# SUTD-MDQS/QILaplace.jl

Measured on AMD Instinct MI355X. Metric: MPO×MPS site-contractions/sec + max |coeff err|, n=24 χ_s=64 χ_c=128, higher is better.
Workload: dtype f64; 1 GPU; zt_n24_chi64_D128; sites=48, mps_bonds_max=64, mpo_bonds_max=128, parallelism=replicas x1 (one signal per GPU), ranks_reported_by_collective_backend=1

## Files before the change

### qilaplace.jl_amd/csrc/qil_internal.h

```cpp
#pragma once

#include <hip/hip_runtime.h>
#include <hip/hip_complex.h>

#include <cstdint>
#include <cstdio>
#include <cstring>
#include <functional>
#include <map>
#include <condition_variable>
#include <mutex>
#include <set>
#include <string>
#include <vector>

#include "qilaplace_hip.h"
#include "qilaplace_hip_testing.h"

#include <atomic>

struct qil_lds_grant {
    static constexpr int kDevices = 64;
    std::atomic<size_t> bytes[kDevices] = {};
    hipError_t ensure(int device, const void* fn, size_t want) {
// ... 125 lines not shown
void qil_comm_orphan(struct qil_comm* cm);
void qil_ctx_transfer(qil_context* from, qil_context* to, void* p);
void qil_chain_rebind(struct qil_chain* c, qil_context* to);
int qil_mps_clone_to(qil_context* ctx, const struct qil_mps* psi, struct qil_mps** out);

static inline size_t qil_elem_size(int dtype) { return dtype == QIL_C64 ? 16 : 8; }

struct qil_chain {
    qil_context* ctx = nullptr;
    int dtype = QIL_F64;
    int paired = 0;
    int phys_rank = 1;
    std::vector<int64_t> dims;
    std::vector<int64_t> site_ids;
    std::vector<void*> site;
    double amplitude = 1.0;
    qil_chain() = default;
    qil_chain(const qil_chain&) = delete;
    qil_chain& operator=(const qil_chain&) = delete;
    ~qil_chain() {
        if (ctx) ctx->chains.erase(this);
    }
    int64_t n() const { return (int64_t)site.size(); }
    int64_t site_elems(int64_t i) const {
        return dims[i] * (phys_rank == 1 ? 2 : 4) * dims[i + 1];
    }
    size_t site_bytes(int64_t i) const { return (size_t)site_elems(i) * qil_elem_size(dtype); }
};
struct qil_mps : qil_chain {};
struct qil_mpo : qil_chain {};

int qil_chain_alloc(qil_context* ctx, qil_chain* c, int64_t n, int dtype, int paired, int phys_rank,
                    const int64_t* bond_dims, const int64_t* site_ids);
int qil_chain_release(qil_chain* c);
void qil_chain_bind(qil_chain* c, qil_context* ctx);
int qil_chain_set_site(qil_chain* c, int64_t i, void* p, int64_t dl, int64_t dr);
void qil_chain_adopt(qil_chain* c, int64_t i, void* p);

unsigned qil_fail_count();
struct qil_call_scope {
    qil_context* ctx;
    uint64_t serial0;
    unsigned fails0;
    explicit qil_call_scope(qil_context* c);
    ~qil_call_scope();
    qil_call_scope(const qil_call_scope&) = delete;
    qil_call_scope& operator=(const qil_call_scope&) = delete;
};

int qil_dev_right_envs(const struct qil_mps* psi, const char* verb, void** Rall, std::vector<long long>& roff, double* log_norm2);

int qil_dev_gemm(qil_context* ctx, int dtype, int opA, int opB, int64_t m, int64_t n, int64_t k,
                 const void* A, int64_t lda, const void* B, int64_t ldb, void* C, int64_t ldc);
int qil_dev_gemm_skinny(qil_context* ctx, int dtype, int opA, int opB, int64_t m, int64_t n, int64_t k,
                        const void* A, int64_t lda, const void* B, int64_t ldb, void* C, int64_t ldc);
struct qil_gemm_batch {
    int64_t count = 1;
    int64_t a_bs = 0, b_bs = 0, c_bs = 0;
    const uint8_t* b_sel = nullptr;
    int64_t b_sel_step = 0, b_sel_stride = 0;
};
int qil_dev_gemm_batched(qil_context* ctx, int dtype, int opA, int opB, int64_t m, int64_t n, int64_t k,
                         const void* A, int64_t lda, const void* B, int64_t ldb, void* C, int64_t ldc,
                         const qil_gemm_batch* batch);
struct qil_gemm_problem {
    const void* A;
    const void* B;
    void* C;
    int m, n, k;
    int lda, ldb, ldc;
    int tile_begin;
    int pad;
};
int qil_dev_gemm_grouped(qil_context* ctx, int dtype, std::vector<qil_gemm_problem>& probs);
bool qil_dev_gemm_grouped_fits(size_t nproblems);
int qil_check_pair(const char* verb, const struct qil_mps* phi, const struct qil_mps* psi);
int qil_sum_compress_impl(qil_context* ctx, const struct qil_mps* const* terms, int64_t nb, const double* w, int odt,
                          int64_t maxdim, double tol, int sweeps, int64_t zip_maxdim, struct qil_mps** out);
int qil_dev_diag_abs2(qil_context* ctx, int dtype, const void* R, int64_t ldr, int64_t n, double* host_out);
int qil_dev_transpose(qil_context* ctx, int dtype, int conj, int64_t m, int64_t n, const void* A, int64_t lda,
                      void* At, int64_t ldt);
int qil_dev_svd(qil_context* ctx, int dtype, int64_t m, int64_t n, void* A, int64_t lda, void* U,
                int64_t ldu, double* S_host, void* Vh, int64_t ldvh, double negligible_rel = 0.0);
int qil_dev_svd_left(qil_context* ctx, int dtype, int64_t p, int64_t q, void* B, int64_t ldb, void* Uiso, int64_t ldu,
                     double* S_host, void* SVh, int64_t ldsvh, double negligible_rel, int* handled, double cert_cutoff = 0.0,
                     double deflate = 0.0);
int qil_dev_qr_certified(qil_context* ctx, int dtype, int64_t m, int64_t n, const void* A, int64_t lda, double cutoff, void* Qout,
                         void* Rout, bool* certified);
int qil_dev_set_identity(qil_context* ctx, int dtype, void* V, int64_t ldv, int64_t n);
int qil_dev_qr_positive(qil_context* ctx, int dtype, int64_t m, int64_t n, void* A, int64_t lda,
                        void* R, int64_t ldr, bool orthonormal = false);
int qil_dev_copy2d(qil_context* ctx, void* dst, size_t dpitch, const void* src, size_t spitch, size_t width, size_t height);
int qil_dev_copy(qil_context* ctx, void* dst, const void* src, size_t bytes);
int qil_dev_zero2d(qil_context* ctx, void* dst, size_t pitch, size_t width, size_t height);
int qil_dev_zero(qil_context* ctx, void* dst, size_t bytes);
int64_t qil_truncation_rank(const double* S, int64_t n, double cutoff, bool use_cutoff, int64_t maxdim,
                            int64_t mindim);
int qil_dev_scale(qil_context* ctx, int dtype, int side, int64_t m, int64_t n, void* A, int64_t lda,
                  const double* s_host);
int qil_dev_fill_normal(qil_context* ctx, int dtype, void* p, int64_t n_elems, uint64_t seed,
                        double scale);
```

### qilaplace.jl_amd/csrc/qil_linalg.hip

```cpp
#include <algorithm>
#include <chrono>
#include <cmath>
#include <cstring>
#include <numeric>
#include <utility>

#include "qil_internal.h"
#include "qil_launch.h"
#include "qil_device_utils.h"

namespace {

using namespace qil_dev;

constexpr int GK = 16;
#ifndef QIL_GEMM_GAUSS
#define QIL_GEMM_GAUSS 1
#endif
#ifndef QIL_GEMM_PAD
#define QIL_GEMM_PAD 2
#endif
constexpr int GPAD = QIL_GEMM_PAD;
typedef double d4 __attribute__((ext_vector_type(4)));

__device__ __forceinline__ void put_plane(double* S0, double* S1, int off, double v) {
    S0[off] = v;
    (void)S1;
}
__device__ __forceinline__ void put_plane(double* S0, double* S1, int off, c64 v) {
    S0[off] = v.re;
    S1[off] = v.im;
}
__device__ __forceinline__ double maybe_conj(double v, int) { return v; }
__device__ __forceinline__ c64 maybe_conj(c64 v, int cj) { return cj ? c64{v.re, -v.im} : v; }

template <class T, int BM, int BN, int WM, int WN, bool PIPE, bool ARC, bool BKC, int GKT = GK, int DEEP = 0>
__device__ __forceinline__ void gemm_mfma_body(const uint3 blockIdx, const uint3 gridDim, long long m, long long n, long long k_total,
                                                 const T* __restrict__ A, long long a_rs, long long a_ks, int conjA,
                                                 const T* __restrict__ B, long long b_ks, long long b_cs, int conjB,
                                                 T* __restrict__ C, long long ldc, long long kchunk,
                                                 long long cstride, int tiles_m, int tiles_n, int col_fastest,
                                                 long long a_bs, long long b_bs, long long c_bs,
                                                 const int* __restrict__ cmap, int cmap_blk,
                                                 const uint8_t* __restrict__ b_sel, long long b_sel_step,
                                                 long long b_sel_stride, int subtract) {
    constexpr bool CX = sizeof(T) == 16;
    constexpr int NP = CX ? 2 : 1;
    constexpr int LA = BM + GPAD, LB = BN + GPAD;
    constexpr int NBUF = PIPE ? 2 : 1;
    constexpr int TM = WM / 16, TN = WN / 16;
    constexpr int EA = BM * GKT / 256, EB = BN * GKT / 256;
    static_assert((BM / WM) * (BN / WN) == 4, "4 waves per workgroup");
    extern __shared__ __attribute__((aligned(16))) char gemm_smem[];
    double* As = reinterpret_cast<double*>(gemm_smem);
    double* Bs = As + NBUF * NP * GKT * LA;
    const int tid = threadIdx.x;
    const int lane = tid & 63, wave = tid >> 6;
    const int wr = (wave % (BM / WM)) * WM, wc = (wave / (BM / WM)) * WN;
    const int l15 = lane & 15, l4 = lane >> 4;
    int tile = blockIdx.x;
    if (col_fastest & 2) tile = (tile % 8) * (tiles_m * tiles_n / 8) + tile / 8;
    int tm, tn;
    if (col_fastest & 1) {
        tn = tile % tiles_n;
        tm = tile / tiles_n;
    } else {
        tm = tile % tiles_m;
        tn = tile / tiles_m;
    }
    const long long row0 = (long long)tm * BM, col0 = (long long)tn * BN;
    const long long kbeg = (long long)blockIdx.z * kchunk;
    const long long kend = min(k_total, kbeg + kchunk);
    A += (long long)blockIdx.y * a_bs;
    B += (long long)blockIdx.y * b_bs;
    if (b_sel) B += (long long)b_sel[(long long)blockIdx.y * b_sel_step] * b_sel_stride;
    C += (long long)blockIdx.z * cstride + (long long)blockIdx.y * c_bs;
    if (cmap) cmap += (long long)blockIdx.y * (n / cmap_blk);

    d4 rr[TM][TN], ii[CX ? TM : 1][CX ? TN : 1], ri[CX ? TM : 1][CX ? TN : 1];
#pragma unroll
    for (int a = 0; a < TM; ++a)
#pragma unroll
        for (int b = 0; b < TN; ++b) {
            rr[a][b] = d4{0, 0, 0, 0};
            if (CX) {
                ii[a][b] = d4{0, 0, 0, 0};
                ri[a][b] = d4{0, 0, 0, 0};
            }
        }
    constexpr bool a_rows_contig = ARC, b_k_contig = BKC;
    T ra[EA], rb[EB];
    const T* pa[EA];
    const T* pb[EB];
    int ka[EA], kb[EB], sa[EA], sb[EB];
#pragma unroll
    for (int e = 0; e < EA; ++e) {
        const int idx = tid + 256 * e;
        const int i = a_rows_contig ? idx % BM : idx / GKT;
// ... 90 lines not shown
                for (int ti = 0; ti < TM; ++ti)
#pragma unroll
                    for (int tj = 0; tj < TN; ++tj) {
                        rr[ti][tj] = __builtin_amdgcn_mfma_f64_16x16x4f64(bre[tj], are[ti], rr[ti][tj], 0, 0, 0);
                        if constexpr (CX) {
                            ii[ti][tj] = __builtin_amdgcn_mfma_f64_16x16x4f64(bim[tj], aim[ti], ii[ti][tj], 0, 0, 0);
                            ri[ti][tj] = __builtin_amdgcn_mfma_f64_16x16x4f64(bim[tj], are[ti], ri[ti][tj], 0, 0, 0);
                            ri[ti][tj] = __builtin_amdgcn_mfma_f64_16x16x4f64(bre[tj], aim[ti], ri[ti][tj], 0, 0, 0);
                        }
                    }
            }
        }
    };
    if constexpr (PIPE && DEEP) {
        T ra1[EA], rb1[EB];
        if (kbeg < kend) load_tile_into(ra, rb, kbeg);
        if (kbeg + GKT < kend) load_tile_into(ra1, rb1, kbeg + GKT);
        for (long long k0 = kbeg; k0 < kend; k0 += 2 * GKT) {
            store_tile_from(ra, rb, 0, k0);
            __syncthreads();
            if (k0 + 2 * GKT < kend) load_tile_into(ra, rb, k0 + 2 * GKT);
            mfma_tile(0);
            if (k0 + GKT >= kend) break;
            store_tile_from(ra1, rb1, 1, k0 + GKT);
            __syncthreads();
            if (k0 + 3 * GKT < kend) load_tile_into(ra1, rb1, k0 + 3 * GKT);
            mfma_tile(1);
        }
    } else {
        int buf = 0;
        if (PIPE && kbeg < kend) load_tile(kbeg);
        for (long long k0 = kbeg; k0 < kend; k0 += GKT) {
            if (!PIPE) {
                if (k0 > kbeg) __syncthreads();
                load_tile(k0);
            }
            store_tile(buf, k0);
            __syncthreads();
            if (PIPE && k0 + GKT < kend) load_tile(k0 + GKT);
            mfma_tile(buf);
            if (PIPE) buf ^= 1;
        }
    }
#pragma unroll
    for (int ti = 0; ti < TM; ++ti)
#pragma unroll
        for (int tj = 0; tj < TN; ++tj)
#pragma unroll
            for (int r = 0; r < 4; ++r) {
                const long long gr = row0 + wr + 16 * ti + l15;
                const long long gc = col0 + wc + 16 * tj + l4 + 4 * r;
                if (gr < m && gc < n) {
                    const long long oc = cmap ? (long long)cmap[gc / cmap_blk] * cmap_blk + gc % cmap_blk : gc;
                    double* cp = reinterpret_cast<double*>(C + gr + ldc * oc);
                    if (subtract) {
                        if (CX) {
                            cp[0] -= rr[ti][tj][r] - ii[ti][tj][r];
                            cp[1] -= QIL_GEMM_GAUSS ? rr[ti][tj][r] + ri[ti][tj][r] : ri[ti][tj][r];
                        } else {
                            cp[0] -= rr[ti][tj][r];
                        }
                    } else if (CX) {
                        cp[0] = rr[ti][tj][r] - ii[ti][tj][r];
                        cp[1] = QIL_GEMM_GAUSS ? rr[ti][tj][r] + ri[ti][tj][r] : ri[ti][tj][r];
                    } else {
                        cp[0] = rr[ti][tj][r];
                    }
                }
            }
}
template <class T, int BM, int BN, int WM, int WN, bool PIPE, bool ARC, bool BKC, int GKT = GK, int DEEP = 0>
struct gemm_mfma_k {
    static constexpr int NT = 256, MINW = (DEEP ? 1 : (BM * BN <= 128 * 128 ? 2 : 1));
    template <class... QA>
    static __device__ __forceinline__ void run(const uint3 b, const uint3 g, QA... a) {
        gemm_mfma_body<T, BM, BN, WM, WN, PIPE, ARC, BKC, GKT, DEEP>(b, g, a...);
    }
};

template <class T>
__device__ __forceinline__ void splitk_reduce_body(const uint3 blockIdx, const uint3 gridDim, const T* __restrict__ W, long long cstride, int splits, long long m, long long n,
                              T* __restrict__ C, long long ldc, int subtract) {
    for (long long t = blockIdx.x * (long long)blockDim.x + threadIdx.x; t < m * n;
         t += (long long)gridDim.x * blockDim.x) {
        T acc = W[t];
        for (int z = 1; z < splits; ++z) acc = add_t(acc, W[t + z * cstride]);
        T* cp = C + (t % m) + ldc * (t / m);
        *cp = subtract ? sub_t(*cp, acc) : acc;
    }
}
template <class T>
struct splitk_reduce_k {
    static constexpr int NT = 1024, MINW = 1;
    template <class... QA>
    static __device__ __forceinline__ void run(const uint3 b, const uint3 g, QA... a) {
        splitk_reduce_body<T>(b, g, a...);
    }
};

struct gemm_batch {
    int count = 1;
    long long a_bs = 0, b_bs = 0, c_bs = 0;
    const int* cmap = nullptr;
    int cmap_blk = 1;
    const uint8_t* b_sel = nullptr;
    long long b_sel_step = 0, b_sel_stride = 0;
    int subtract = 0;
// ... 88 lines not shown
        QIL_TRY(qil_ctx_alloc(ctx, (size_t)(cstride * splits) * sizeof(T), &wsp));
        Cout = static_cast<T*>(wsp);
        ldo = m;
    }
    const int order = p.col_fastest | (p.xcd ? 2 : 0);
#define QIL_GEMM_K(ARCv, BKCv)                                                                                               \
    QIL_TRY((qil_klaunch<gemm_mfma_k<T, BM, BN, WM, WN, PIPE, ARCv, BKCv, GKT, DEEP>>(                                                      \
        ctx, dim3((unsigned)tiles, (unsigned)bt.count, (unsigned)splits), dim3(256), lds, m, n, k, A, a_rs, a_ks, conjA, B, b_ks, \
        b_cs, conjB, Cout, ldo, (long long)p.kchunk, cstride, (int)p.tiles_m, (int)p.tiles_n, order, bt.a_bs, bt.b_bs, c_bs, bt.cmap,  \
        bt.cmap_blk, bt.b_sel, bt.b_sel_step, bt.b_sel_stride, splits > 1 ? 0 : bt.subtract)))
    if (p.arc && p.bkc) QIL_GEMM_K(true, true);
    else if (p.arc) QIL_GEMM_K(true, false);
    else if (p.bkc) QIL_GEMM_K(false, true);
    else QIL_GEMM_K(false, false);
#undef QIL_GEMM_K
    if (splits > 1) {
        QIL_TRY((qil_klaunch<splitk_reduce_k<T>>(ctx, dim3((unsigned)std::min<long long>((cstride + 255) / 256, 2048)), dim3(256), 0, (const T*)Cout, cstride, splits, m, n * bt.count, C, ldc, bt.subtract)));
        QIL_HIP(hipGetLastError());
        qil_ctx_free(ctx, wsp);
    }
    return QIL_OK;
}

template <class T>
int gemm_dispatch(qil_context* ctx, int opA, int opB, long long m, long long n, long long k, const T* A,
                  long long lda, const T* B, long long ldb, T* C, long long ldc,
                  const gemm_batch& batch = gemm_batch{}) {
    if (m == 0 || n == 0) return QIL_OK;
    QIL_REQUIRE(opA >= 0 && opA <= 3 && opB >= 0 && opB <= 3, QIL_EINVAL_ARG, "gemm: bad op codes %d, %d", opA, opB);
    const bool at = opA == 1 || opA == 2, bt = opB == 1 || opB == 2;
    const long long a_rs = at ? lda : 1, a_ks = at ? 1 : lda;
    const long long b_ks = bt ? ldb : 1, b_cs = bt ? 1 : ldb;
    const int cA = (opA == 2 || opA == 3) ? 1 : 0, cB = (opB == 2 || opB == 3) ? 1 : 0;
    constexpr bool CX = sizeof(T) == 16;
    qil_gemm_plan_info p;
    const int si = gemm_plan(CX, opA, opB, m, n, k, lda, ldb, ldc, batch.count, batch.c_bs, batch.cmap != nullptr, batch.skinny_m, &p);
#define QIL_GEMM_GO(SI) \
    case SI: return gemm_launch<T, SI>(ctx, p, m, n, k, A, a_rs, a_ks, cA, B, b_ks, b_cs, cB, C, ldc, batch)
    switch (si) {
        QIL_GEMM_GO(GS_32x64_DEEP);
        QIL_GEMM_GO(GS_48x64_DEEP);
        QIL_GEMM_GO(GS_32x32);
        QIL_GEMM_GO(GS_64x64);
    }
    if constexpr (!CX) {
        switch (si) {
            QIL_GEMM_GO(GS_64x144);
            QIL_GEMM_GO(GS_128x128);
            QIL_GEMM_GO(GS_128x64);
        }
    }
#undef QIL_GEMM_GO
    return qil_fail(QIL_EINVAL_ARG, "gemm: no kernel for tile shape %d", si);
}

template <class T>
__device__ __forceinline__ void jacobi_round_body(const uint3 blockIdx, const uint3 gridDim, T* __restrict__ A, long long lda, long long m,
                                                    T* __restrict__ V, long long ldv, int vrows, int n,
                                                    int npad, int round, double tol,
                                                    int* __restrict__ rotated,
                                                    const double* __restrict__ negligible) {
    __shared__ double red[16];
    const int i = blockIdx.x;
    int p, q;
    if (i == 0) {
        p = npad - 1;
        q = round;
    } else {
        p = (round + i) % (npad - 1);
        q = (round + npad - 1 - i) % (npad - 1);
    }
    if (p >= n || q >= n) return;
    if (p > q) {
        const int t = p;
        p = q;
        q = t;
    }
    T* ap = A + lda * p;
    T* aq = A + lda * q;
    double v[4] = {0, 0, 0, 0};
    for (long long r = threadIdx.x; r < m; r += 256) {
        const T x = ap[r], y = aq[r];
        v[0] += abs2_t(x);
        v[1] += abs2_t(y);
        dot_parts(x, y, v[2], v[3]);
    }
    block_sum<4>(v, red);
    if (negligible) {
        const double ng = *negligible;
        if (v[0] < ng || v[1] < ng) return;
    }
    double c, s, pr, pi;
    bool big;
    if (!jacobi_rotation<sizeof(T) == 16>(v[0], v[1], v[2], v[3], tol, c, s, pr, pi, big)) return;
    if (threadIdx.x == 0) {
        rotated[0] = 1;
        if (big) rotated[1] = 1;
    }
    for (long long r = threadIdx.x; r < m; r += 256) {
        T x = ap[r], y = aq[r];
        rotate_pair(x, y, c, s, pr, pi);
        ap[r] = x;
        aq[r] = y;
    }
    T* vp = V + ldv * p;
    T* vq = V + ldv * q;
// ... 3503 lines not shown
    if (!words || width * height > ((size_t)64 << 20)) {
        QIL_HIP(hipMemset2DAsync(dst, pitch, 0, width, height, qil_stream(ctx)));
        return QIL_OK;
    }
    const long long total = (long long)(width / 4) * (long long)height;
    return qil_klaunch<zero2d_k>(ctx, dim3((unsigned)std::min<long long>((total + 255) / 256, 2048)), dim3(256), 0,
                                 static_cast<unsigned*>(dst), (long long)(pitch / 4), (long long)(width / 4), (long long)height);
}
int qil_dev_zero(qil_context* ctx, void* dst, size_t bytes) { return qil_dev_zero2d(ctx, dst, bytes, bytes, 1); }

namespace {

template <class T>
__device__ __forceinline__ void scale_kernel_body(const uint3 blockIdx, const uint3 gridDim, T* __restrict__ A, long long lda, long long m, long long n,
                             const double* __restrict__ s, int side) {
    const long long total = m * n;
    for (long long t = blockIdx.x * (long long)blockDim.x + threadIdx.x; t < total;
         t += (long long)gridDim.x * blockDim.x) {
        const long long i = t % m, j = t / m;
        A[i + lda * j] = scale_t(A[i + lda * j], side ? s[j] : s[i]);
    }
}
template <class T>
struct scale_kernel_k {
    static constexpr int NT = 1024, MINW = 1;
    template <class... QA>
    static __device__ __forceinline__ void run(const uint3 b, const uint3 g, QA... a) {
        scale_kernel_body<T>(b, g, a...);
    }
};

__global__ void fill_normal_kernel(double* __restrict__ p, long long n, uint64_t seed, double scale) {
    for (long long t = blockIdx.x * (long long)blockDim.x + threadIdx.x; t < n;
         t += (long long)gridDim.x * blockDim.x) {
        const uint64_t h1 = splitmix64(seed ^ splitmix64(2ull * (uint64_t)t));
        const uint64_t h2 = splitmix64(seed ^ splitmix64(2ull * (uint64_t)t + 1ull));
        const double u1 = ((double)(h1 >> 11) + 1.0) * (1.0 / 9007199254740993.0);
        const double u2 = (double)(h2 >> 11) * (1.0 / 9007199254740992.0);
        p[t] = scale * sqrt(-2.0 * log(u1)) * cospi(2.0 * u2);
    }
}

}

int qil_dev_gemm(qil_context* ctx, int dtype, int opA, int opB, int64_t m, int64_t n, int64_t k,
                 const void* A, int64_t lda, const void* B, int64_t ldb, void* C, int64_t ldc) {
    if (dtype == QIL_C64)
        return gemm_dispatch<c64>(ctx, opA, opB, m, n, k, (const c64*)A, lda, (const c64*)B, ldb, (c64*)C, ldc);
    static const int real_op[4] = {0, 1, 1, 0};
    return gemm_dispatch<double>(ctx, real_op[opA & 3], real_op[opB & 3], m, n, k, (const double*)A, lda,
                                 (const double*)B, ldb, (double*)C, ldc);
}

int qil_dev_gemm_skinny(qil_context* ctx, int dtype, int opA, int opB, int64_t m, int64_t n, int64_t k,
                        const void* A, int64_t lda, const void* B, int64_t ldb, void* C, int64_t ldc) {
    gemm_batch bt;
    bt.skinny_m = 1;
    if (dtype == QIL_C64)
        return gemm_dispatch<c64>(ctx, opA, opB, m, n, k, (const c64*)A, lda, (const c64*)B, ldb, (c64*)C, ldc, bt);
    static const int real_op[4] = {0, 1, 1, 0};
    return gemm_dispatch<double>(ctx, real_op[opA & 3], real_op[opB & 3], m, n, k, (const double*)A, lda,
                                 (const double*)B, ldb, (double*)C, ldc, bt);
}

static int gemm_check_args(int opA, int opB, int64_t m, int64_t n, int64_t k, int64_t lda, int64_t ldb, int64_t ldc) {
    QIL_REQUIRE(m >= 1 && n >= 1 && k >= 1, QIL_EINVAL_ARG, "gemm: empty operand");
    QIL_REQUIRE(opA >= 0 && opA <= 3 && opB >= 0 && opB <= 3, QIL_EINVAL_ARG, "gemm: bad op code");
    const int64_t a_rows = (opA == 0 || opA == 3) ? m : k, b_rows = (opB == 0 || opB == 3) ? k : n;
    QIL_REQUIRE(lda >= a_rows, QIL_EINVAL_ARG, "gemm: lda %lld is smaller than the %lld stored rows of A", (long long)lda, (long long)a_rows);
    QIL_REQUIRE(ldb >= b_rows, QIL_EINVAL_ARG, "gemm: ldb %lld is smaller than the %lld stored rows of B", (long long)ldb, (long long)b_rows);
    QIL_REQUIRE(ldc >= m, QIL_EINVAL_ARG, "gemm: ldc %lld is smaller than the %lld rows of C", (long long)ldc, (long long)m);
    return QIL_OK;
}

extern "C" int qil_gemm(qil_context* ctx, int dtype, int opA, int opB, int64_t m, int64_t n, int64_t k,
                        const void* A, int64_t lda, const void* B, int64_t ldb, void* C, int64_t ldc) {
    QIL_REQUIRE(ctx && A && B && C, QIL_EINVAL_ARG, "gemm: null argument");
    QIL_TRY(gemm_check_args(opA, opB, m, n, k, lda, ldb, ldc));
    QIL_TRY(qil_ctx_activate(ctx));
    qil_call_scope call_scope(ctx);
    const size_t e = qil_elem_size(dtype);
    const int64_t a_cols = (opA == 0 || opA == 3) ? k : m, b_cols = (opB == 0 || opB == 3) ? n : k;
    void *dA = nullptr, *dB = nullptr, *dC = nullptr;
    QIL_TRY(qil_ctx_alloc(ctx, (size_t)(lda * a_cols) * e, &dA));
    QIL_TRY(qil_ctx_alloc(ctx, (size_t)(ldb * b_cols) * e, &dB));
    QIL_TRY(qil_ctx_alloc(ctx, (size_t)(ldc * n) * e, &dC));
    QIL_HIP(hipMemcpyAsync(dA, A, (size_t)(lda * a_cols) * e, hipMemcpyHostToDevice, qil_stream(ctx)));
    QIL_HIP(hipMemcpyAsync(dB, B, (size_t)(ldb * b_cols) * e, hipMemcpyHostToDevice, qil_stream(ctx)));
    QIL_TRY(qil_dev_zero(ctx, dC, (size_t)(ldc * n) * e));
    QIL_HIP(qil_stream_sync(ctx));
    QIL_TRY(qil_dev_gemm(ctx, dtype, opA, opB, m, n, k, dA, lda, dB, ldb, dC, ldc));
    QIL_TRY(qil_read_back(ctx, C, dC, (size_t)(ldc * n) * e));
    qil_ctx_free(ctx, dA);
    qil_ctx_free(ctx, dB);
    qil_ctx_free(ctx, dC);
    return QIL_OK;
}

extern "C" int qil_gemm_plan(int dtype, int opA, int opB, int64_t m, int64_t n, int64_t k, int64_t lda, int64_t ldb, int64_t ldc,
                             int64_t count, int64_t c_bs, int has_cmap, int skinny_m, qil_gemm_plan_info* plan) {
    QIL_REQUIRE(plan, QIL_EINVAL_ARG, "gemm: null argument");
    QIL_REQUIRE(dtype == QIL_F64 || dtype == QIL_C64, QIL_EINVAL_ARG, "gemm: bad dtype %d", dtype);
    QIL_TRY(gemm_check_args(opA, opB, m, n, k, lda, ldb, ldc));
    QIL_REQUIRE(count >= 1 && count <= 65535, QIL_EINVAL_ARG, "gemm: batch count %lld exceeds the grid limit", (long long)count);
    static const int real_op[4] = {0, 1, 1, 0};
    if (dtype == QIL_F64) opA = real_op[opA], opB = real_op[opB];
    gemm_plan(dtype == QIL_C64, opA, opB, m, n, k, lda, ldb, ldc, count, c_bs, has_cmap != 0, skinny_m, plan);
    return QIL_OK;
}

extern "C" int qil_gemm_batched_host(qil_context* ctx, int dtype, int opA, int opB, int64_t m, int64_t n, int64_t k,
                                     const qil_gemm_host_operand* A, const qil_gemm_host_operand* B, const qil_gemm_host_operand* C,
                                     int64_t count, int subtract, int skinny_m, const uint8_t* b_sel, int64_t b_sel_step,
                                     int64_t b_sel_stride, const int32_t* cmap, int64_t cmap_blk) {
    QIL_REQUIRE(ctx && A && B && C && A->base && B->base && C->base, QIL_EINVAL_ARG, "gemm: null argument");
// ... 310 lines not shown
```

### qilaplace.jl_amd/csrc/qil_readout.hip

```cpp
#include "qil_internal.h"
#include "qil_launch.h"
#include "qil_device_utils.h"
#include <set>
#include <mutex>
#include <map>

namespace {

using namespace qil_dev;

__device__ __forceinline__ double shfl_xor_t(double v, int m) { return __shfl_xor(v, m, 64); }
__device__ __forceinline__ c64 shfl_xor_t(c64 v, int m) {
    return c64{__shfl_xor(v.re, m, 64), __shfl_xor(v.im, m, 64)};
}
__device__ __forceinline__ double one_t(double) { return 1.0; }
__device__ __forceinline__ c64 one_t(c64) { return c64{1.0, 0.0}; }

struct ChainSite {
    const void* A;
    const void* W;
    int cl, cr, Dl, Dr;
};

constexpr int kThreads = 256;
// ... 72 lines not shown
        __syncthreads();
        const long long n2 = (long long)S.cr * S.Dr;
        for (long long t = threadIdx.x; t < n2; t += kThreads) {
            const int beta = (int)(t % S.cr);
            const int b = (int)(t / S.cr);
            c64 acc{};
            for (int sp = 0; sp < 2; ++sp) {
                const c64* x = X + sp * msz + (long long)S.cl * b;
                const TA* acol = A + (long long)S.cl * (sp + 2LL * beta);
                for (int alpha = 0; alpha < S.cl; ++alpha) acc = cmul_add(acc, x[alpha], acol[alpha]);
            }
            Mn[beta + (long long)S.cr * b] = acc;
        }
        __threadfence_block();
        __syncthreads();
        c64* t = M;
        M = Mn;
        Mn = t;
    }
    if (threadIdx.x == 0) out[q] = c64{M[0].re * amplitude, M[0].im * amplitude};
}

template <class T>
__global__ void select_slice(const T* __restrict__ Tm, long long nb, int cr, const uint8_t* __restrict__ bits,
                             int n, int site, T* __restrict__ Vn) {
    const long long total = nb * cr;
    for (long long t = blockIdx.x * (long long)blockDim.x + threadIdx.x; t < total;
         t += (long long)gridDim.x * blockDim.x) {
        const long long q = t % nb;
        const long long beta = t / nb;
        const int bit = bits[q * n + site];
        Vn[t] = bit == 2 ? add_t(Tm[q + nb * (2 * beta)], Tm[q + nb * (1 + 2 * beta)])
                         : Tm[q + nb * (bit + 2 * beta)];
    }
}

template <class T>
__device__ __forceinline__ void select_slice_body(const uint3 blockIdx, const uint3 gridDim, const T* __restrict__ Tm, long long nb, int cr,
                                                  const uint8_t* __restrict__ bits, int n, int site, T* __restrict__ Vn) {
    const long long total = nb * cr;
    for (long long t = blockIdx.x * (long long)blockDim.x + threadIdx.x; t < total; t += (long long)gridDim.x * blockDim.x) {
        const long long q = t % nb;
        const long long beta = t / nb;
        const int bit = bits[q * n + site];
        Vn[t] = bit == 2 ? add_t(Tm[q + nb * (2 * beta)], Tm[q + nb * (1 + 2 * beta)]) : Tm[q + nb * (bit + 2 * beta)];
    }
}
template <class T>
struct select_slice_k {
    static constexpr int NT = 256, MINW = 1;
    template <class... QA>
    static __device__ __forceinline__ void run(const uint3 b, const uint3 g, QA... a) {
        select_slice_body<T>(b, g, a...);
    }
};
template <class T>
__device__ __forceinline__ void gather_rows_body(const uint3 blockIdx, const uint3 gridDim, const T* __restrict__ Tm, long long nb, int cr,
                                                 const int* __restrict__ map, T* __restrict__ Vn) {
    const long long total = nb * cr;
    for (long long t = blockIdx.x * (long long)blockDim.x + threadIdx.x; t < total; t += (long long)gridDim.x * blockDim.x) {
        const long long r = t % nb, beta = t / nb;
        Vn[t] = Tm[map[r] + nb * beta];
    }
}
template <class T>
struct gather_rows_k {
    static constexpr int NT = 256, MINW = 1;
    template <class... QA>
    static __device__ __forceinline__ void run(const uint3 b, const uint3 g, QA... a) {
        gather_rows_body<T>(b, g, a...);
    }
};
template <class T>
__device__ __forceinline__ void fill_ones_body(const uint3 blockIdx, const uint3 gridDim, T* __restrict__ v, long long n) {
    for (long long t = blockIdx.x * (long long)blockDim.x + threadIdx.x; t < n; t += (long long)gridDim.x * blockDim.x) v[t] = one_t(T{});
}
template <class T>
struct fill_ones_k {
    static constexpr int NT = 256, MINW = 1;
    template <class... QA>
    static __device__ __forceinline__ void run(const uint3 b, const uint3 g, QA... a) {
        fill_ones_body<T>(b, g, a...);
    }
};
template <class T>
__device__ __forceinline__ void finish_coeff_body(const uint3 blockIdx, const uint3 gridDim, const T* __restrict__ v, long long nb,
                                                  double amplitude, c64* __restrict__ out) {
    for (long long t = blockIdx.x * (long long)blockDim.x + threadIdx.x; t < nb; t += (long long)gridDim.x * blockDim.x) {
        const c64 r = to_c64(v[t]);
        out[t] = c64{r.re * amplitude, r.im * amplitude};
    }
}
template <class T>
struct finish_coeff_k {
    static constexpr int NT = 256, MINW = 1;
    template <class... QA>
    static __device__ __forceinline__ void run(const uint3 b, const uint3 g, QA... a) {
        finish_coeff_body<T>(b, g, a...);
    }
};

template <class T>
__global__ void fill_ones(T* __restrict__ v, long long n) {
    for (long long t = blockIdx.x * (long long)blockDim.x + threadIdx.x; t < n;
         t += (long long)gridDim.x * blockDim.x)
        v[t] = one_t(T{});
}

template <class T>
__global__ void finish_coeff(const T* __restrict__ v, long long nb, double amplitude, c64* __restrict__ out) {
    for (long long t = blockIdx.x * (long long)blockDim.x + threadIdx.x; t < nb;
         t += (long long)gridDim.x * blockDim.x) {
        const c64 r = to_c64(v[t]);
        out[t] = c64{r.re * amplitude, r.im * amplitude};
    }
}


template <class T>
__global__ void slice_sum(const T* __restrict__ A, int cl, int cr, T* __restrict__ out) {
    const long long total = (long long)cl * cr;
    for (long long t = blockIdx.x * (long long)blockDim.x + threadIdx.x; t < total; t += (long long)gridDim.x * blockDim.x) {
        const int al = (int)(t % cl);
// ... 127 lines not shown
int upload_bits(qil_context* ctx, int64_t nb, int64_t n, const uint8_t* bits, uint8_t** dbits, int max_bit = 1) {
    for (int64_t t = 0; t < nb * n; ++t)
        QIL_REQUIRE(bits[t] <= max_bit, QIL_EINVAL_CONFIG, "coefficient: bit value %d outside [0,%d]", (int)bits[t],
                    max_bit);
    void* p = nullptr;
    QIL_TRY(qil_ctx_alloc(ctx, (size_t)(nb * n), &p));
    hipError_t e = hipMemcpyAsync(p, bits, (size_t)(nb * n), hipMemcpyHostToDevice, qil_stream(ctx));
    if (e == hipSuccess) e = qil_stream_sync(ctx);
    if (e != hipSuccess) {
        qil_ctx_free(ctx, p);
        return qil_fail(QIL_EHIP, "bit upload failed: %s", hipGetErrorString(e));
    }
    *dbits = static_cast<uint8_t*>(p);
    return QIL_OK;
}

}

static int coefficient_impl(const qil_mps* psi, int64_t nb, const uint8_t* bits, double* out, int max_bit);

extern "C" int qil_coefficient_batch(const qil_mps* psi, int64_t nb, const uint8_t* bits, double* out) {
    return coefficient_impl(psi, nb, bits, out, 1);
}

extern "C" int qil_coefficient_marginal_batch(const qil_mps* psi, int64_t nb, const uint8_t* bits, double* out) {
    return coefficient_impl(psi, nb, bits, out, 2);
}

struct SortPlan {
    int* dmap = nullptr;
    std::vector<int64_t> n0;
};
static int build_sort_plan(qil_context* ctx, int64_t nb, int64_t n, const uint8_t* bits, SortPlan* plan) {
    std::vector<int> map((size_t)(n * nb)), order((size_t)nb), next((size_t)nb), pos((size_t)nb);
    plan->n0.assign((size_t)n, 0);
    auto order_of = [&](int64_t site, std::vector<int>& o) -> int64_t {
        int64_t z = 0;
        if (site >= n) {
            for (int64_t q = 0; q < nb; ++q) o[(size_t)q] = (int)q;
            return nb;
        }
        for (int64_t q = 0; q < nb; ++q)
            if (bits[q * n + site] == 0) o[(size_t)z++] = (int)q;
        int64_t w = z;
        for (int64_t q = 0; q < nb; ++q)
            if (bits[q * n + site] != 0) o[(size_t)w++] = (int)q;
        return z;
    };
    plan->n0[0] = order_of(0, order);
    for (int64_t i = 0; i < n; ++i) {
        for (int64_t r = 0; r < nb; ++r) pos[(size_t)order[(size_t)r]] = (int)r;
        const int64_t z = order_of(i + 1, next);
        if (i + 1 < n) plan->n0[(size_t)i + 1] = z;
        for (int64_t r = 0; r < nb; ++r) map[(size_t)(i * nb + r)] = pos[(size_t)next[(size_t)r]];
        order.swap(next);
    }
    void* p = nullptr;
    QIL_TRY(qil_ctx_alloc(ctx, map.size() * sizeof(int), &p));
    hipError_t e = hipMemcpyAsync(p, map.data(), map.size() * sizeof(int), hipMemcpyHostToDevice, qil_stream(ctx));
    if (e == hipSuccess) e = qil_stream_sync(ctx);
    if (e != hipSuccess) {
        qil_ctx_free(ctx, p);
        return qil_fail(QIL_EHIP, "read-out plan upload failed: %s", hipGetErrorString(e));
    }
    plan->dmap = static_cast<int*>(p);
    return QIL_OK;
}
static bool wants_sort_plan(const qil_mps* psi, int64_t nb, int max_bit) {
    if (max_bit > 1 || nb < 4) return false;
    long long maxchi = 1;
    for (int64_t i = 0; i < psi->n(); ++i) maxchi = std::max<long long>(maxchi, psi->dims[(size_t)i + 1]);
    return maxchi >= 128 || (nb >= 1024 && maxchi >= 16);
}

static int coefficient_enqueue(const qil_mps* psi, int64_t nb, const uint8_t* dbits, void* dout, const SortPlan* plan = nullptr) {
    qil_context* ctx = psi->ctx;
    const int64_t n = psi->n();
    std::vector<ChainSite> tab((size_t)n);
    long long maxchi = 1;
    for (int64_t i = 0; i < n; ++i) {
        tab[(size_t)i] = ChainSite{psi->site[(size_t)i], nullptr, (int)psi->dims[(size_t)i],
                                   (int)psi->dims[(size_t)i + 1], 1, 1};
        maxchi = std::max<long long>(maxchi, psi->dims[(size_t)i + 1]);
    }
    const size_t esz = qil_elem_size(psi->dtype);
    static const long long min_chi = 128;
    if (nb >= 4 && (maxchi >= min_chi || (nb >= 1024 && maxchi >= 16))) {
        void *V = nullptr, *Vn = nullptr, *Tm = nullptr;
        QIL_TRY(qil_ctx_alloc(ctx, (size_t)(nb * maxchi) * esz, &V));
        QIL_TRY(qil_ctx_alloc(ctx, (size_t)(nb * maxchi) * esz, &Vn));
        QIL_TRY(qil_ctx_alloc(ctx, (size_t)(2 * nb * maxchi) * esz, &Tm));
        const bool cx = psi->dtype == QIL_C64;
        const unsigned g1 = (unsigned)std::min<long long>((nb + 255) / 256, 4096);
        if (cx) QIL_TRY((qil_klaunch<fill_ones_k<c64>>(ctx, dim3(g1), dim3(256), 0, (c64*)V, (long long)nb)));
        else QIL_TRY((qil_klaunch<fill_ones_k<double>>(ctx, dim3(g1), dim3(256), 0, (double*)V, (long long)nb)));
        for (int64_t i = 0; i < n; ++i) {
            const int64_t cl = psi->dims[(size_t)i], cr = psi->dims[(size_t)i + 1];
            const unsigned g = (unsigned)std::min<long long>((nb * cr + 255) / 256, 65536);
            if (plan && plan->dmap) {
                const int64_t z = plan->n0[(size_t)i];
                const char* site = static_cast<const char*>(psi->site[(size_t)i]);
                for (int sl = 0; sl < 2; ++sl) {
                    const int64_t r0 = sl ? z : 0, rows = sl ? nb - z : z;
                    if (rows == 0) continue;
                    const void* Vs = static_cast<const char*>(V) + (size_t)r0 * esz;
                    void* Ts = static_cast<char*>(Tm) + (size_t)r0 * esz;
                    const void* As = site + (size_t)(sl * cl) * esz;
                    if (rows <= 48) QIL_TRY(qil_dev_gemm_skinny(ctx, psi->dtype, 0, 0, rows, cr, cl, Vs, nb, As, 2 * cl, Ts, nb));
                    else QIL_TRY(qil_dev_gemm(ctx, psi->dtype, 0, 0, rows, cr, cl, Vs, nb, As, 2 * cl, Ts, nb));
                }
                const int* map = plan->dmap + (size_t)(i * nb);
                if (cx) QIL_TRY((qil_klaunch<gather_rows_k<c64>>(ctx, dim3(g), dim3(256), 0, (const c64*)Tm, (long long)nb, (int)cr, map, (c64*)Vn)));
                else QIL_TRY((qil_klaunch<gather_rows_k<double>>(ctx, dim3(g), dim3(256), 0, (const double*)Tm, (long long)nb, (int)cr, map, (double*)Vn)));
                std::swap(V, Vn);
                continue;
            }
            QIL_TRY(qil_dev_gemm(ctx, psi->dtype, 0, 0, nb, 2 * cr, cl, V, nb, psi->site[(size_t)i], cl, Tm, nb));
            if (cx)
                QIL_TRY((qil_klaunch<select_slice_k<c64>>(ctx, dim3(g), dim3(256), 0, (const c64*)Tm, (long long)nb, (int)cr,
                                                          (const uint8_t*)dbits, (int)n, (int)i, (c64*)Vn)));
            else
                QIL_TRY((qil_klaunch<select_slice_k<double>>(ctx, dim3(g), dim3(256), 0, (const double*)Tm, (long long)nb, (int)cr,
                                                             (const uint8_t*)dbits, (int)n, (int)i, (double*)Vn)));
            std::swap(V, Vn);
        }
        if (cx) QIL_TRY((qil_klaunch<finish_coeff_k<c64>>(ctx, dim3(g1), dim3(256), 0, (const c64*)V, (long long)nb, psi->amplitude, (c64*)dout)));
        else QIL_TRY((qil_klaunch<finish_coeff_k<double>>(ctx, dim3(g1), dim3(256), 0, (const double*)V, (long long)nb, psi->amplitude, (c64*)dout)));
        qil_ctx_free(ctx, V);
        qil_ctx_free(ctx, Vn);
        qil_ctx_free(ctx, Tm);
        return QIL_OK;
    }
    void *scratch = nullptr, *pin = nullptr, *dtab = nullptr;
    int slot = 0;
    QIL_TRY(qil_ctx_alloc(ctx, (size_t)(2 * nb * maxchi) * esz, &scratch));
    QIL_TRY(qil_ctx_desc_acquire(ctx, tab.size() * sizeof(ChainSite), &pin, &dtab, &slot));
    memcpy(pin, tab.data(), tab.size() * sizeof(ChainSite));
    QIL_HIP(hipMemcpyAsync(dtab, pin, tab.size() * sizeof(ChainSite), hipMemcpyHostToDevice, qil_stream(ctx)));
    if (psi->dtype == QIL_C64)
        hipLaunchKernelGGL(coefficient_chain<c64>, dim3((unsigned)nb), dim3(kThreads), 0, qil_stream(ctx),
                           (const ChainSite*)dtab, (int)n, dbits, (c64*)scratch, maxchi, (c64*)dout,
                           psi->amplitude);
    else
        hipLaunchKernelGGL(coefficient_chain<double>, dim3((unsigned)nb), dim3(kThreads), 0, qil_stream(ctx),
                           (const ChainSite*)dtab, (int)n, dbits, (double*)scratch, maxchi, (c64*)dout,
                           psi->amplitude);
    QIL_HIP(hipGetLastError());
    QIL_TRY(qil_ctx_desc_commit(ctx, slot));
    qil_ctx_free(ctx, scratch);
    return QIL_OK;
}

static int coefficient_impl(const qil_mps* psi, int64_t nb, const uint8_t* bits, double* out, int max_bit) {
    QIL_REQUIRE(psi && (nb == 0 || (bits && out)), QIL_EINVAL_ARG, "coefficient: null argument");
    if (nb == 0) return QIL_OK;
    qil_context* ctx = psi->ctx;
    QIL_TRY(qil_ctx_activate(ctx));
    qil_call_scope call_scope(ctx);
    uint8_t* dbits = nullptr;
    QIL_TRY(upload_bits(ctx, nb, psi->n(), bits, &dbits, max_bit));
    SortPlan plan;
    if (wants_sort_plan(psi, nb, max_bit)) QIL_TRY(build_sort_plan(ctx, nb, psi->n(), bits, &plan));
    void* dout = nullptr;
    QIL_TRY(qil_ctx_alloc(ctx, (size_t)nb * 16, &dout));
    QIL_TRY(coefficient_enqueue(psi, nb, dbits, dout, &plan));
    if (plan.dmap) qil_ctx_free(ctx, plan.dmap);
    QIL_HIP(hipMemcpyAsync(out, dout, (size_t)nb * 16, hipMemcpyDeviceToHost, qil_stream(ctx)));
    QIL_HIP(qil_stream_sync(ctx));
    qil_ctx_free(ctx, dout);
    qil_ctx_free(ctx, dbits);
    return QIL_OK;
}

int qil_apply_coefficient_sweep_dev(const qil_mpo* const* Ws, int64_t nw, const qil_mps* psi, int64_t nb, const uint8_t* bits,
                                    void* dout) {
    qil_context* ctx = psi->ctx;
    uint8_t* dbits = nullptr;
    QIL_TRY(upload_bits(ctx, nb, psi->n(), bits, &dbits, 1));
    SortPlan plan;
    if (nb >= 4) QIL_TRY(build_sort_plan(ctx, nb, psi->n(), bits, &plan));
    bool distinct = true;
    {
        std::set<const qil_mpo*> seen;
// ... 212 lines not shown
```

Baseline: 3935 site-contractions/s.

## Fuse readout split GEMMs and row gather into one row-scatter GEMM launch

In the sorted readout path, the two per-slice GEMMs plus a separate gather kernel are replaced by one launch that runs both row halves as grid.y slices and writes outputs directly to permuted rows through an inverted row map. This removes the Tm intermediate buffer, its extra write and read, and several launches per site. Split-K cases fall back to a workspace plus a reduce kernel that scatters rows. Fusion only happens when the two halves pick compatible tile shapes, and can be turned off with an environment variable.

```diff
diff --git a/qilaplace.jl_amd/csrc/qil_internal.h b/qilaplace.jl_amd/csrc/qil_internal.h
--- a/qilaplace.jl_amd/csrc/qil_internal.h
+++ b/qilaplace.jl_amd/csrc/qil_internal.h
@@ -201,8 +201,8 @@
 
 int qil_dev_gemm(qil_context* ctx, int dtype, int opA, int opB, int64_t m, int64_t n, int64_t k,
                  const void* A, int64_t lda, const void* B, int64_t ldb, void* C, int64_t ldc);
-int qil_dev_gemm_skinny(qil_context* ctx, int dtype, int opA, int opB, int64_t m, int64_t n, int64_t k,
-                        const void* A, int64_t lda, const void* B, int64_t ldb, void* C, int64_t ldc);
+int qil_dev_gemm_rows_scatter(qil_context* ctx, int dtype, int64_t m0, int64_t m1, int64_t n, int64_t k, const void* A, int64_t lda,
+                              const void* B0, const void* B1, int64_t ldb, void* C, int64_t ldc, const int* rmap);
 struct qil_gemm_batch {
     int64_t count = 1;
     int64_t a_bs = 0, b_bs = 0, c_bs = 0;
diff --git a/qilaplace.jl_amd/csrc/qil_linalg.hip b/qilaplace.jl_amd/csrc/qil_linalg.hip
--- a/qilaplace.jl_amd/csrc/qil_linalg.hip
+++ b/qilaplace.jl_amd/csrc/qil_linalg.hip
@@ -43,7 +43,8 @@
                                                  long long a_bs, long long b_bs, long long c_bs,
                                                  const int* __restrict__ cmap, int cmap_blk,
                                                  const uint8_t* __restrict__ b_sel, long long b_sel_step,
-                                                 long long b_sel_stride, int subtract) {
+                                                 long long b_sel_stride, int subtract,
+                                                 const int* __restrict__ rmap = nullptr) {
     constexpr bool CX = sizeof(T) == 16;
     constexpr int NP = CX ? 2 : 1;
     constexpr int LA = BM + GPAD, LB = BN + GPAD;
@@ -240,7 +241,8 @@
                 const long long gc = col0 + wc + 16 * tj + l4 + 4 * r;
                 if (gr < m && gc < n) {
                     const long long oc = cmap ? (long long)cmap[gc / cmap_blk] * cmap_blk + gc % cmap_blk : gc;
-                    double* cp = reinterpret_cast<double*>(C + gr + ldc * oc);
+                    const long long orow = rmap ? (long long)rmap[gr] : gr;
+                    double* cp = reinterpret_cast<double*>(C + orow + ldc * oc);
                     if (subtract) {
                         if (CX) {
                             cp[0] -= rr[ti][tj][r] - ii[ti][tj][r];
@@ -435,6 +437,158 @@
     }
 #undef QIL_GEMM_GO
     return qil_fail(QIL_EINVAL_ARG, "gemm: no kernel for tile shape %d", si);
+}
+
+struct gemm_rows_half {
+    const void* A;
+    const void* B;
+    void* W;
+    const int* rmap;
+    long long m, kchunk;
+    int tiles_m, tiles_n, order, splits;
+};
+struct gemm_rows_args {
+    long long n, k, lda, ldb, ldc;
+    void* C;
+    gemm_rows_half h[2];
+};
+template <class T, int SI0, int SI1>
+struct gemm_rows_k {
+    static constexpr gemm_shape S0 = GEMM_SHAPES[SI0], S1 = GEMM_SHAPES[SI1];
+    static constexpr int NT = 256;
+    static constexpr int MINW = (S0.deep || S1.deep) ? 1 : (S0.bm * S0.bn <= 128 * 128 && S1.bm * S1.bn <= 128 * 128 ? 2 : 1);
+    template <int SI>
+    static __device__ __forceinline__ void half(const uint3 b, const uint3 g, const gemm_rows_args& a, const gemm_rows_half& h) {
+        constexpr gemm_shape S = GEMM_SHAPES[SI];
+        T* C = static_cast<T*>(h.W ? h.W : a.C);
+        gemm_mfma_body<T, S.bm, S.bn, S.wm, S.wn, true, true, true, S.gkt, S.deep>(
+            b, g, h.m, a.n, a.k, static_cast<const T*>(h.A), 1LL, a.lda, 0, static_cast<const T*>(h.B), 1LL, a.ldb, 0, C,
+            h.W ? h.m : a.ldc, h.kchunk, h.W ? h.m * a.n : 0LL, h.tiles_m, h.tiles_n, h.order, 0LL, 0LL, 0LL, nullptr, 1, nullptr,
+            0LL, 0LL, 0, h.W ? nullptr : h.rmap);
+    }
+    static __device__ __forceinline__ void run(const uint3 b, const uint3 g, gemm_rows_args a) {
+        const gemm_rows_half h = b.y ? a.h[1] : a.h[0];
+        if (b.x >= (unsigned)(h.tiles_m * h.tiles_n) || b.z >= (unsigned)h.splits) return;
+        const uint3 bb = make_uint3(b.x, 0u, b.z);
+        if (SI0 == SI1 || b.y == 0) half<SI0>(bb, g, a, h);
+        else half<SI1>(bb, g, a, h);
+    }
+};
+template <class T>
+struct gemm_rows_reduce_k {
+    static constexpr int NT = 1024, MINW = 1;
+    static __device__ __forceinline__ void run(const uint3 blockIdx, const uint3 gridDim, gemm_rows_args a, int nh) {
+        const long long m0 = a.h[0].m, m1 = nh > 1 ? a.h[1].m : 0, mt = m0 + m1;
+        const T* __restrict__ W0 = static_cast<const T*>(a.h[0].W);
+        const T* __restrict__ W1 = static_cast<const T*>(a.h[1].W);
+        const int* __restrict__ rm0 = a.h[0].rmap;
+        const int* __restrict__ rm1 = a.h[1].rmap;
+        const int sp0 = a.h[0].splits, sp1 = a.h[1].splits;
+        T* __restrict__ C = static_cast<T*>(a.C);
+        for (long long t = blockIdx.x * (long long)blockDim.x + threadIdx.x; t < mt * a.n; t += (long long)gridDim.x * blockDim.x) {
+            const long long r = t % mt, c = t / mt;
+            const bool lo = r < m0;
+            const T* W = lo ? W0 : W1;
+            if (!W) continue;
+            const long long lr = lo ? r : r - m0, m = lo ? m0 : m1, cstride = m * a.n;
+            const int splits = lo ? sp0 : sp1;
+            W += lr + m * c;
+            T acc = W[0];
+            for (int z = 1; z < splits; ++z) acc = add_t(acc, W[z * cstride]);
+            C[(lo ? rm0 : rm1)[lr] + a.ldc * c] = acc;
+        }
+    }
+};
+
+template <class T>
+int gemm_rows_launch(qil_context* ctx, gemm_rows_args a, int nh, const int* si) {
+    constexpr bool CX = sizeof(T) == 16;
+    constexpr int NP = CX ? 2 : 1;
+    size_t lds = 0, wsz = 0;
+    unsigned gx = 0, gz = 0;
+    for (int h = 0; h < nh; ++h) {
+        const gemm_shape& s = GEMM_SHAPES[si[h]];
+        lds = std::max(lds, (size_t)2 * NP * s.gkt * ((s.bm + GPAD) + (s.bn + GPAD)) * sizeof(double));
+        gx = std::max(gx, (unsigned)(a.h[h].tiles_m * a.h[h].tiles_n));
+        gz = std::max(gz, (unsigned)a.h[h].splits);
+        if (a.h[h].splits > 1) wsz += (size_t)(a.h[h].m * a.n * a.h[h].splits);
+    }
+    void* wsp = nullptr;
+    if (wsz) {
+        QIL_TRY(qil_ctx_alloc(ctx, wsz * sizeof(T), &wsp));
+        T* w = static_cast<T*>(wsp);
+        for (int h = 0; h < nh; ++h)
+            if (a.h[h].splits > 1) {
+                a.h[h].W = w;
+                w += a.h[h].m * a.n * a.h[h].splits;
+            }
+    }
+    if (nh == 1) a.h[1] = a.h[0];
+    const dim3 grid(gx, (unsigned)nh, gz);
+    const int s0 = si[0], s1 = nh > 1 ? si[1] : si[0];
+    int st = -1;
+#define QIL_ROWS_GO(A0, A1) \
+    if (s0 == A0 && s1 == A1) st = qil_klaunch<gemm_rows_k<T, A0, A1>>(ctx, grid, dim3(256), lds, a)
+    QIL_ROWS_GO(GS_32x64_DEEP, GS_32x64_DEEP);
+    QIL_ROWS_GO(GS_32x64_DEEP, GS_48x64_DEEP);
+    QIL_ROWS_GO(GS_48x64_DEEP, GS_48x64_DEEP);
+    QIL_ROWS_GO(GS_32x32, GS_32x32);
+    QIL_ROWS_GO(GS_64x64, GS_64x64);
+    if constexpr (!CX) {
+        QIL_ROWS_GO(GS_64x144, GS_64x144);
+        QIL_ROWS_GO(GS_128x128, GS_128x128);
+        QIL_ROWS_GO(GS_128x64, GS_128x64);
+    }
+#undef QIL_ROWS_GO
+    if (st == -1) st = qil_fail(QIL_EINVAL_ARG, "gemm: no row-scatter kernel for tile shapes %d, %d", s0, s1);
+    if (st == QIL_OK && wsz) {
+        const long long total = (a.h[0].m + (nh > 1 ? a.h[1].m : 0)) * a.n;
+        st = qil_klaunch<gemm_rows_reduce_k<T>>(ctx, dim3((unsigned)std::min<long long>((total + 255) / 256, 2048)), dim3(256), 0, a, nh);
+    }
+    if (wsp) qil_ctx_free(ctx, wsp);
+    return st;
+}
+
+bool gemm_rows_fusable(int s0, int s1) {
+    return s0 == s1 || (std::min(s0, s1) == GS_32x64_DEEP && std::max(s0, s1) == GS_48x64_DEEP);
+}
+
+template <class T>
+int gemm_rows_scatter(qil_context* ctx, long long m0, long long m1, long long n, long long k, const T* A, long long lda, const T* B0,
+                      const T* B1, long long ldb, T* C, long long ldc, const int* rmap) {
+    constexpr bool CX = sizeof(T) == 16;
+    if (n == 0) return QIL_OK;
+    const bool fuse = !(getenv("QIL_READOUT_FUSE") && atoi(getenv("QIL_READOUT_FUSE")) == 0);
+    gemm_rows_args a;
+    a.n = n, a.k = k, a.lda = lda, a.ldb = ldb, a.ldc = ldc, a.C = C;
+    const long long ms[2] = {m0, m1}, r0[2] = {0, m0};
+    const T* Bs[2] = {B0, B1};
+    int si[2] = {0, 0}, nh = 0;
+    bool skinny[2] = {false, false};
+    for (int h = 0; h < 2; ++h) {
+        if (ms[h] == 0) continue;
+        qil_gemm_plan_info p;
+        skinny[nh] = ms[h] <= 48;
+        si[nh] = gemm_plan(CX, 0, 0, ms[h], n, k, lda, ldb, ldc, 1, 0, false, skinny[nh] ? 1 : 0, &p);
+        gemm_rows_half& g = a.h[nh];
+        g.A = A + r0[h], g.B = Bs[h], g.W = nullptr, g.rmap = rmap + r0[h];
+        g.m = ms[h], g.kchunk = p.kchunk;
+        g.tiles_m = (int)p.tiles_m, g.tiles_n = (int)p.tiles_n, g.order = p.col_fastest | (p.xcd ? 2 : 0), g.splits = p.splits;
+        ++nh;
+    }
+    if (nh == 2 && fuse && skinny[0] == skinny[1] && gemm_rows_fusable(si[0], si[1])) {
+        if (si[0] > si[1]) {
+            std::swap(si[0], si[1]);
+            std::swap(a.h[0], a.h[1]);
+        }
+        return gemm_rows_launch<T>(ctx, a, 2, si);
+    }
+    for (int h = 0; h < nh; ++h) {
+        gemm_rows_args one = a;
+        one.h[0] = a.h[h];
+        QIL_TRY(gemm_rows_launch<T>(ctx, one, 1, si + h));
+    }
+    return QIL_OK;
 }
 
 template <class T>
@@ -4044,15 +4198,11 @@
                                  (const double*)B, ldb, (double*)C, ldc);
 }
 
-int qil_dev_gemm_skinny(qil_context* ctx, int dtype, int opA, int opB, int64_t m, int64_t n, int64_t k,
-                        const void* A, int64_t lda, const void* B, int64_t ldb, void* C, int64_t ldc) {
-    gemm_batch bt;
-    bt.skinny_m = 1;
+int qil_dev_gemm_rows_scatter(qil_context* ctx, int dtype, int64_t m0, int64_t m1, int64_t n, int64_t k, const void* A, int64_t lda,
+                              const void* B0, const void* B1, int64_t ldb, void* C, int64_t ldc, const int* rmap) {
     if (dtype == QIL_C64)
-        return gemm_dispatch<c64>(ctx, opA, opB, m, n, k, (const c64*)A, lda, (const c64*)B, ldb, (c64*)C, ldc, bt);
-    static const int real_op[4] = {0, 1, 1, 0};
-    return gemm_dispatch<double>(ctx, real_op[opA & 3], real_op[opB & 3], m, n, k, (const double*)A, lda,
-                                 (const double*)B, ldb, (double*)C, ldc, bt);
+        return gemm_rows_scatter<c64>(ctx, m0, m1, n, k, (const c64*)A, lda, (const c64*)B0, (const c64*)B1, ldb, (c64*)C, ldc, rmap);
+    return gemm_rows_scatter<double>(ctx, m0, m1, n, k, (const double*)A, lda, (const double*)B0, (const double*)B1, ldb, (double*)C, ldc, rmap);
 }
 
 static int gemm_check_args(int opA, int opB, int64_t m, int64_t n, int64_t k, int64_t lda, int64_t ldb, int64_t ldc) {
diff --git a/qilaplace.jl_amd/csrc/qil_readout.hip b/qilaplace.jl_amd/csrc/qil_readout.hip
--- a/qilaplace.jl_amd/csrc/qil_readout.hip
+++ b/qilaplace.jl_amd/csrc/qil_readout.hip
@@ -148,23 +148,6 @@
     template <class... QA>
     static __device__ __forceinline__ void run(const uint3 b, const uint3 g, QA... a) {
         select_slice_body<T>(b, g, a...);
-    }
-};
-template <class T>
-__device__ __forceinline__ void gather_rows_body(const uint3 blockIdx, const uint3 gridDim, const T* __restrict__ Tm, long long nb, int cr,
-                                                 const int* __restrict__ map, T* __restrict__ Vn) {
-    const long long total = nb * cr;
-    for (long long t = blockIdx.x * (long long)blockDim.x + threadIdx.x; t < total; t += (long long)gridDim.x * blockDim.x) {
-        const long long r = t % nb, beta = t / nb;
-        Vn[t] = Tm[map[r] + nb * beta];
-    }
-}
-template <class T>
-struct gather_rows_k {
-    static constexpr int NT = 256, MINW = 1;
-    template <class... QA>
-    static __device__ __forceinline__ void run(const uint3 b, const uint3 g, QA... a) {
-        gather_rows_body<T>(b, g, a...);
     }
 };
 template <class T>
@@ -398,7 +381,7 @@
         for (int64_t r = 0; r < nb; ++r) pos[(size_t)order[(size_t)r]] = (int)r;
         const int64_t z = order_of(i + 1, next);
         if (i + 1 < n) plan->n0[(size_t)i + 1] = z;
-        for (int64_t r = 0; r < nb; ++r) map[(size_t)(i * nb + r)] = pos[(size_t)next[(size_t)r]];
+        for (int64_t r = 0; r < nb; ++r) map[(size_t)(i * nb + pos[(size_t)next[(size_t)r]])] = (int)r;
         order.swap(next);
     }
     void* p = nullptr;
@@ -432,35 +415,26 @@
     const size_t esz = qil_elem_size(psi->dtype);
     static const long long min_chi = 128;
     if (nb >= 4 && (maxchi >= min_chi || (nb >= 1024 && maxchi >= 16))) {
+        const bool sorted = plan && plan->dmap;
         void *V = nullptr, *Vn = nullptr, *Tm = nullptr;
         QIL_TRY(qil_ctx_alloc(ctx, (size_t)(nb * maxchi) * esz, &V));
         QIL_TRY(qil_ctx_alloc(ctx, (size_t)(nb * maxchi) * esz, &Vn));
-        QIL_TRY(qil_ctx_alloc(ctx, (size_t)(2 * nb * maxchi) * esz, &Tm));
+        if (!sorted) QIL_TRY(qil_ctx_alloc(ctx, (size_t)(2 * nb * maxchi) * esz, &Tm));
         const bool cx = psi->dtype == QIL_C64;
         const unsigned g1 = (unsigned)std::min<long long>((nb + 255) / 256, 4096);
         if (cx) QIL_TRY((qil_klaunch<fill_ones_k<c64>>(ctx, dim3(g1), dim3(256), 0, (c64*)V, (long long)nb)));
         else QIL_TRY((qil_klaunch<fill_ones_k<double>>(ctx, dim3(g1), dim3(256), 0, (double*)V, (long long)nb)));
         for (int64_t i = 0; i < n; ++i) {
             const int64_t cl = psi->dims[(size_t)i], cr = psi->dims[(size_t)i + 1];
-            const unsigned g = (unsigned)std::min<long long>((nb * cr + 255) / 256, 65536);
-            if (plan && plan->dmap) {
+            if (sorted) {
                 const int64_t z = plan->n0[(size_t)i];
                 const char* site = static_cast<const char*>(psi->site[(size_t)i]);
-                for (int sl = 0; sl < 2; ++sl) {
-                    const int64_t r0 = sl ? z : 0, rows = sl ? nb - z : z;
-                    if (rows == 0) continue;
-                    const void* Vs = static_cast<const char*>(V) + (size_t)r0 * esz;
-                    void* Ts = static_cast<char*>(Tm) + (size_t)r0 * esz;
-                    const void* As = site + (size_t)(sl * cl) * esz;
-                    if (rows <= 48) QIL_TRY(qil_dev_gemm_skinny(ctx, psi->dtype, 0, 0, rows, cr, cl, Vs, nb, As, 2 * cl, Ts, nb));
-                    else QIL_TRY(qil_dev_gemm(ctx, psi->dtype, 0, 0, rows, cr, cl, Vs, nb, As, 2 * cl, Ts, nb));
-                }
-                const int* map = plan->dmap + (size_t)(i * nb);
-                if (cx) QIL_TRY((qil_klaunch<gather_rows_k<c64>>(ctx, dim3(g), dim3(256), 0, (const c64*)Tm, (long long)nb, (int)cr, map, (c64*)Vn)));
-                else QIL_TRY((qil_klaunch<gather_rows_k<double>>(ctx, dim3(g), dim3(256), 0, (const double*)Tm, (long long)nb, (int)cr, map, (double*)Vn)));
+                QIL_TRY(qil_dev_gemm_rows_scatter(ctx, psi->dtype, z, nb - z, cr, cl, V, nb, site, site + (size_t)cl * esz, 2 * cl, Vn, nb,
+                                                  plan->dmap + (size_t)(i * nb)));
                 std::swap(V, Vn);
                 continue;
             }
+            const unsigned g = (unsigned)std::min<long long>((nb * cr + 255) / 256, 65536);
             QIL_TRY(qil_dev_gemm(ctx, psi->dtype, 0, 0, nb, 2 * cr, cl, V, nb, psi->site[(size_t)i], cl, Tm, nb));
             if (cx)
                 QIL_TRY((qil_klaunch<select_slice_k<c64>>(ctx, dim3(g), dim3(256), 0, (const c64*)Tm, (long long)nb, (int)cr,
@@ -474,7 +448,7 @@
         else QIL_TRY((qil_klaunch<finish_coeff_k<double>>(ctx, dim3(g1), dim3(256), 0, (const double*)V, (long long)nb, psi->amplitude, (c64*)dout)));
         qil_ctx_free(ctx, V);
         qil_ctx_free(ctx, Vn);
-        qil_ctx_free(ctx, Tm);
+        if (Tm) qil_ctx_free(ctx, Tm);
         return QIL_OK;
     }
     void *scratch = nullptr, *pin = nullptr, *dtab = nullptr;
```

Result: slower. 3753 site-contractions/s (-4.6%).
